# srsampson/SingleCarrier

Measured on AMD Instinct MI355X. Metric: demodulated Msamples/sec (whole node), 65536-channel 8 kHz batch; BER vs ref, higher is better.
Workload: dtype f32

## Files before the change

profiles/stamps.py:

```python
import ctypes as C
import json
import os
import sys

import numpy as np

ROOT = os.path.dirname(os.path.dirname(os.path.abspath(__file__)))
sys.path.insert(0, ROOT)
import singlecarrier_amd as sc

mode = sys.argv[1] if len(sys.argv) > 1 else "both"
if mode == "front":
    os.environ["QPSK_ABLATE"] = "front"
sc.LIB_PATH = os.path.join(ROOT, "singlecarrier_amd", "csrc", "build", "libqpsk_hip_stamps.so")
lib = sc.lib()
lib.qpsk_debug_stamps.argtypes = [C.c_void_p, C.c_int]
import torch

nch, nf = 65536, 32
x = torch.from_numpy(sc.synth(3, nch, nf)).cuda()
bits = torch.empty((nch, nf, 62), dtype=torch.uint8, device="cuda")
valid = torch.empty((nch, nf), dtype=torch.uint8, device="cuda")
rx = sc.Receiver(nch)
rx.demod_device(x, bits, valid)
torch.cuda.synchronize()
st = np.zeros(16, np.uint64)
lib.qpsk_debug_stamps(st.ctypes.data, 1)
rx.demod_device(x, bits, valid)
torch.cuda.synchronize()
lib.qpsk_debug_stamps(st.ctypes.data, 1)
names = {0: "mix", 1: "store_window+prefetch+sync", 6: "front_channel+mi+sync (total)",
         7: "frame barrier wait", 8: "FIR decimated (D)", 9: "FIR head (F)+sync",
         10: "T image+sync", 11: "correlate (MFMA)", 12: "argmax (DPP max)"}
bnames = {13: "back: frame (128 train steps + job/outputs)", 14: "back: frame barrier wait"}
ch_iters = nch * nf
waves = nch // 32
out = {"mode": mode, "cycles_per_channel": {}}
tot = sum(int(st[i]) for i in (0, 1, 6, 7))
for i, nm in names.items():
    v = int(st[i]) / ch_iters
    out["cycles_per_channel"][nm] = round(v, 1)
out["share_of_loop"] = {names[i]: round(int(st[i]) / tot, 3) for i in (0, 1, 6, 7)}
bw = nch // 64
btot = int(st[13]) + int(st[14])
out["back_cycles_per_frame"] = {bnames[i]: round(int(st[i]) / (bw * nf), 1) for i in (13, 14)}
out["back_share"] = {bnames[i]: round(int(st[i]) / max(btot, 1), 3) for i in (13, 14)}
fr = bw * nf
out["back_alone_tail"] = {
    "frames_back_last_share": round(int(st[5]) / fr, 3),
    "tail_cycles_per_frame_all": round(int(st[15]) / fr, 1),
    "tail_cycles_per_frame_when_last": round(int(st[15]) / max(int(st[5]), 1), 1),
    "frame_cycles": round(btot / fr, 1),
    "tail_share_of_frame": round(int(st[15]) / max(btot, 1), 3)}
print(json.dumps(out, indent=1))
```

singlecarrier_amd/__init__.py:

```python
from __future__ import annotations

import ctypes as C
import os
import subprocess

import numpy as np

HERE = os.path.dirname(os.path.abspath(__file__))
LIB_PATH = os.environ.get("QPSK_LIB") or os.path.join(HERE, "libqpsk_hip.so")

FRAME_SIZE = 1880
DATA_SYMBOLS = 31
PREAMBLE_LENGTH = 128
BITS_PER_FRAME = 496
NBITS = 62
CYCLES = 5

_lib = None


class _CF(C.Structure):
    _fields_ = [("re", C.c_float), ("im", C.c_float)]


class QpskError(RuntimeError):
    code = 0


QPSK_EINVAL, QPSK_ENOMEM, QPSK_ENODEV, QPSK_EBUSY, QPSK_ESTALL = -1, -2, -3, -4, -5


def build(verbose: bool = False) -> str:
    out = subprocess.run(["make", "-C", os.path.join(HERE, "csrc")], capture_output=True,
                         text=True)
    if out.returncode != 0:
        raise QpskError("build failed:\n" + out.stdout[-4000:] + out.stderr[-4000:])
    if verbose:
        print(out.stdout)
    return LIB_PATH


KERNEL_SOURCES = ("qpsk_rx.hip", "qpsk_rx_shared.h", "qpsk_herr.h", "qpsk_rx_dev.h", "qpsk_rx_front.h",
                  "qpsk_rx_back.h", "qpsk_rx_quad.h", "qpsk_hunt.h", "qpsk_rcp.h", "qpsk_consts.h",
                  "qpsk_fft_dev.h", "qpsk_split.h", "Makefile")


def kernel_source_hash(csrc: str = None) -> str:
    csrc = csrc or os.path.join(HERE, "csrc")
    inc = os.path.join(os.path.dirname(HERE), "include")
    out = subprocess.run(["make", "-s", "--no-print-directory", "-C", csrc, "khash", f"INCDIR={inc}"],
                         capture_output=True, text=True)
    if out.returncode != 0:
        raise QpskError("make khash failed:\n" + out.stderr[-2000:])
    return out.stdout.strip()


def kernel_hash() -> str:
    return lib().qpsk_kernel_hash().decode()


def lib():
    global _lib
    if _lib is None:
        if not os.path.exists(LIB_PATH):
            raise QpskError(f"{LIB_PATH} not built: run singlecarrier_amd.build() "
                            "or make -C singlecarrier_amd/csrc")
        try:
            import torch
        except Exception:
            pass
        L = C.CDLL(LIB_PATH)
        vp, i32, u64 = C.c_void_p, C.c_int, C.c_uint64
        L.qpsk_rx_create.restype = vp
        L.qpsk_rx_create.argtypes = [i32, i32, C.POINTER(C.c_int)]
        L.qpsk_rx_create_mode.restype = vp
        L.qpsk_rx_create_mode.argtypes = [i32, i32, i32, C.POINTER(C.c_int)]
        L.qpsk_rx_mode.argtypes = [vp]
        L.qpsk_rx_destroy.argtypes = [vp]
        L.qpsk_rx_reset.argtypes = [vp]
        L.qpsk_rx_channels.argtypes = [vp]
        L.qpsk_rx_frames.restype = u64
        L.qpsk_rx_frames.argtypes = [vp]
        L.qpsk_rx_batch.argtypes = [vp, vp, i32, vp, vp, vp, vp]
        L.qpsk_rx_batch_device.argtypes = [vp, vp, i32, vp, vp, vp, vp, vp]
        L.qpsk_strerror.restype = C.c_char_p
        L.qpsk_strerror.argtypes = [i32]
        L.qpsk_kernel_hash.restype = C.c_char_p
        L.qpsk_kernel_hash.argtypes = []
        L.qpsk_rx_frame.argtypes = [vp, vp]
        L.qpsk_tx_frame.argtypes = [vp, vp, i32, C.c_bool]
        L.qpsk_surface_error.restype = i32
        L.qpsk_rx_timing_enable.argtypes = [vp, i32]
        L.qpsk_rx_sync.argtypes = [vp]
        L.qpsk_rx_timing_collect.argtypes = [vp, C.POINTER(C.c_float), C.POINTER(C.c_int)]
        L.qpsk_rx_timing_split.argtypes = [vp, C.POINTER(C.c_float), C.POINTER(C.c_float),
# ... 432 lines not shown
```

singlecarrier_amd/csrc/qpsk_rx.hip:

```cpp

#if defined(QPSK_FRESH) || defined(QPSK_FRESH_SPLIT) || defined(QPSK_HUNT_MFMA) || \
    defined(QPSK_HUNT_FILTER) || defined(QPSK_HUNT_OVERLAP) || defined(QPSK_FIR_WAIT) || \
    defined(QPSK_FIR_ANCHOR) || defined(QPSK_FIR_SPLIT) || defined(QPSK_SPLIT_BANKS) || \
    defined(QPSK_QDMUL) || defined(QPSK_TRAIN_PRETAB) || defined(QPSK_DYNPRIO) || \
    defined(QPSK_DATA_RING) || defined(QPSK_LATE_YIELD) || defined(QPSK_FB) || defined(QPSK_FB1) || \
    defined(QPSK_ZERO_COPY)
#error "QPSK_FRESH, QPSK_FRESH_SPLIT, QPSK_HUNT_MFMA, QPSK_HUNT_FILTER, QPSK_HUNT_OVERLAP, QPSK_FIR_WAIT, QPSK_FIR_ANCHOR, QPSK_FIR_SPLIT, QPSK_SPLIT_BANKS, QPSK_QDMUL, QPSK_TRAIN_PRETAB, QPSK_DYNPRIO, QPSK_DATA_RING, QPSK_LATE_YIELD, QPSK_FB, QPSK_FB1 and QPSK_ZERO_COPY were removed with their alternative branches: DESIGN.md, Removed knobs, names the commit that still has each"
#endif

#include <hip/hip_runtime.h>

#include <stdint.h>

#include <algorithm>
#include <type_traits>

#include "qpsk_batch.h"
#include "qpsk_consts.h"
#include "qpsk_hunt.h"
#include "qpsk_rx_shared.h"
#include "qpsk_rx_dev.h"
#include "qpsk_rx_front.h"
#include "qpsk_rx_back.h"
#include "qpsk_rx_quad.h"

#pragma clang fp contract(off)

namespace {

#ifndef QPSK_RX_ATTR
#define QPSK_RX_ATTR
#endif
constexpr int kLateYield = 2;

template <int G, bool DUAL, int W, bool QUAD>
constexpr int kBackWavesOf = DUAL ? 2 * G * (QUAD ? W / 16 : 1) : G;

template <int G, int FP, bool DUAL, int W, bool QUAD>
constexpr int kWavesOf = kBackWavesOf<G, DUAL, W, QUAD> + G * FP;

template <int G, int FP, int MODE, bool DUAL, int W = QK_GROUP, bool QUAD = false, bool HP = false>
__global__ void __launch_bounds__((64 * kWavesOf<G, FP, DUAL, W, QUAD>),
                                  ((kWavesOf<G, FP, DUAL, W, QUAD> + 3) / 4)) QPSK_RX_ATTR rx_kernel(
    const int16_t* in, int16_t* hist, const float2* ptab, const unsigned long long* ks,
    float2* win0, float2* win1, int* mi0, int* mi1, int* rt0, int* rt1, uint8_t* bits,
    uint8_t* valid, int32_t* trace, float2* soft, float4* jobs, unsigned* njobs, int nch, int F,
    unsigned g0, int roles, const float* fft_tab, unsigned long long jcap, int* err) {
    static_assert(W == QK_GROUP || (DUAL && G == 1 && W % FP == 0 && W <= QK_GROUP), "group width");
    static_assert(!QUAD || (DUAL && G == 1 && W % 16 == 0), "quad backs: dual chain, one group");
    constexpr int kGroups = G, kFrontPer = FP;
    constexpr int kBackWaves = kBackWavesOf<G, DUAL, W, QUAD>;
    constexpr int kChainWaves = QUAD ? W / 16 : 1;
    constexpr bool kDyn = DUAL && QUAD;
    constexpr int kFrontCh = W / kFrontPer;
    constexpr int kFrontWaves = kGroups * kFrontPer;
    constexpr int kBlock = 64 * kWavesOf<G, FP, DUAL, W, QUAD>;
    const RxArgs a{in, hist, ptab, ks, win0, win1, mi0, mi1, rt0, rt1, bits, valid, trace, soft,
                   jobs, njobs, nch, F, g0, (size_t)jcap, roles, err,
                   HP ? reinterpret_cast<const float2*>(fft_tab) : nullptr};
    __shared__ __attribute__((aligned(16))) float2 P[QK_FRAME];
    constexpr int DM = MODE & 1;
    constexpr int kM = Cfg<DM>::kM, kDecBuf = Cfg<DM>::kDecBuf;
    __shared__ __attribute__((aligned(16))) float2 Ms[kFrontWaves][kM];
    __shared__ __attribute__((aligned(16))) float2 decs[kFrontWaves][kDecBuf][kDec];
    __shared__ int mi_s[kGroups][2][QK_GROUP], rt_s[kGroups][2][QK_GROUP];
    __shared__ __attribute__((aligned(16))) float BT[(MODE & 2) ? kFftHT : kHuntTab];
    constexpr bool kSplitK = MODE == 0 && !HP && !DUAL;
    __shared__ uint32_t p2w[kSplitK ? kSplitTabWords : 1];
    const uint8_t* p2tab = reinterpret_cast<const uint8_t*>(p2w);
    __shared__ int bseq[kGroups][2][kChainWaves], fcnt[kGroups][2][kChainWaves];
    __shared__ int dead_s;
    __shared__ int nwait_s;
#ifdef QPSK_STAMPS
    __shared__ unsigned long long tarr_s[16];
    __shared__ int tsimd_s[16];
#define TAIL_INIT() do { if (lane == 0 && wave < 16) tsimd_s[wave] = (int)((__builtin_amdgcn_s_getreg((31 << 11) | (0 << 6) | 4) >> 4) & 3); } while (0)
#define TAIL_ARRIVE() do { if (lane == 0 && wave < 16) tarr_s[wave] = stamp_now(); } while (0)
#define TAIL_BACK()                                                                           \
    do {                                                                                      \
        unsigned long long tf = 0;                                                            \
        for (int w2 = kBackWaves; w2 < kBackWaves + kFrontWaves && w2 < 16; w2++)             \
            if (tsimd_s[w2] == tsimd_s[wave] && tarr_s[w2] > tf) tf = tarr_s[w2];            \
        if (tf > 0 && tarr_s[wave] > tf) { st_acc[15] += tarr_s[wave] - tf; st_acc[5] += 1; } \
        st_t0 = stamp_now();                                                                  \
    } while (0)
#else
#define TAIL_INIT() do { } while (0)
#define TAIL_ARRIVE() do { } while (0)
#define TAIL_BACK() do { } while (0)
#endif
    if (blockDim.x != (unsigned)kBlock) {
        if (blockIdx.x == 0 && threadIdx.x == 0) atomicOr(err, kErrStall);
        return;
    }
    const int lane = threadIdx.x & 63;
    const int wave = __builtin_amdgcn_readfirstlane(threadIdx.x >> 6);
    const int grp0 = blockIdx.x * kGroups;
    TAIL_INIT();
    for (int i = threadIdx.x; i < QK_FRAME / 2; i += kBlock)
        reinterpret_cast<float4*>(P)[i] = reinterpret_cast<const float4*>(a.ptab)[i];
    if constexpr (kSplitK)
        for (int i = threadIdx.x; i < kSplitTabWords; i += kBlock)
            p2w[i] = reinterpret_cast<const uint32_t*>(&kSplitTab)[i];
    if constexpr ((MODE & 2) != 0) {
        for (int i = threadIdx.x; i < kFftHT; i += kBlock) BT[i] = fft_tab[i];
    } else {
        qhunt::bconst_h_lds(threadIdx.x, kBlock, BT);
    }
    if (wave < kGroups) {
        const int ch = (grp0 + wave) * W + lane;
        if (lane < W && ch < a.nch) {
            mi_s[wave][0][lane] = mi_of(a, a.g0)[ch];
            rt_s[wave][0][lane] = rt_of(a, a.g0)[ch];
        }
    }
    if (threadIdx.x < 2 * kGroups * kChainWaves) (&bseq[0][0][0])[threadIdx.x] = (&fcnt[0][0][0])[threadIdx.x] = 0;
    if (threadIdx.x == 0) dead_s = nwait_s = 0;
    __syncthreads();
    if constexpr (DUAL) {
        constexpr int kBlkCh = W / kChainWaves;
        constexpr int kFrontChB = kBlkCh / kFrontPer;
        static_assert(kBlkCh % kFrontPer == 0, "block split");
        if (wave < kBackWaves) {
            const int gi = (wave >> 1) / kChainWaves;
            const int b = (wave >> 1) % kChainWaves;
            const int sub = QUAD ? lane >> 2 : lane;
            const bool own = sub < kBlkCh;
            const int idx = kBlkCh * b + (own ? sub : 0);
            const int ch = (grp0 + gi) * W + idx;
            const bool live = own && ch < a.nch;
            if (kDyn || roles_prio(a.roles) == kPrioBack) __builtin_amdgcn_s_setprio(2);
            auto poll = [&] {
                if constexpr (kDyn) {
                    const int w = __builtin_amdgcn_readfirstlane(
                        __hip_atomic_load(&nwait_s, __ATOMIC_RELAXED, __HIP_MEMORY_SCOPE_WORKGROUP));
                    if (w > 0) __builtin_amdgcn_s_setprio(0);
                    else __builtin_amdgcn_s_setprio(2);
                }
            };
            if (roles_debug_stall(a.roles) && blockIdx.x == 0 && wave == 0)
                spin_wait(&fcnt[gi][0][0], 1 << 30, a.err, &dead_s, 1u << 12);
            STAMP_DECL
            for (int n = wave & 1; n < a.F; n += 2) {
                const int p = n & 1;
                if (n > 0) {
                    int* const fc = &fcnt[gi][p ^ 1][b];
                    const int need = kFrontPer * ((n - 1) / 2 + 1);
                    if constexpr (kDyn) {
                        const bool waits = __builtin_amdgcn_readfirstlane(__hip_atomic_load(
                                               fc, __ATOMIC_RELAXED, __HIP_MEMORY_SCOPE_WORKGROUP)) < need;
                        if (waits) {
                            __builtin_amdgcn_s_setprio(0);
                            if (lane == 0)
                                __hip_atomic_fetch_add(&nwait_s, 1, __ATOMIC_RELAXED, __HIP_MEMORY_SCOPE_WORKGROUP);
                        }
                        spin_wait(fc, need, a.err, &dead_s);
                        if (waits && lane == 0)
                            __hip_atomic_fetch_add(&nwait_s, -1, __ATOMIC_RELAXED, __HIP_MEMORY_SCOPE_WORKGROUP);
                    } else {
                        spin_wait(fc, need, a.err, &dead_s);
                    }
                }
                STAMP(14);
                const int mi = mi_s[gi][p][idx];
                auto get_rt = [&] {
                    STAMP(13);
                    if (n > 0) spin_wait(&bseq[gi][p ^ 1][b], (n - 1) / 2 + 1, a.err, &dead_s);
                    STAMP(15);
                    return rt_s[gi][p][idx];
                };
                const float2* wn = win_of(a, a.g0 + (unsigned)n) + (size_t)(live ? ch : 0) * kWinStride;
                int* rtn = own ? &rt_s[gi][p ^ 1][idx] : nullptr;
                if constexpr (QUAD)
                    back_frame_quad(a, live ? ch : 0, live, n, mi, get_rt, wn, rtn, poll);
                else
                    back_frame(a, live ? ch : 0, live, n, mi, get_rt, wn, rtn, poll);
                signal_add(&bseq[gi][p][b], 1, lane);
                STAMP(13);
            }
            STAMP_FLUSH();
        } else {
            const int f = wave - kBackWaves;
            const int gi = f / kFrontPer;
            const int fl = f % kFrontPer;
            const int split = (kGroups == 1 && kChainWaves == 1) ? roles_split(a.roles) : 0;
            auto share = [&](int x) { return ((x + kBackWaves) & 3) < kBackWaves; };
            int cbeg = 0;
            for (int x = 0; x < fl; x++) cbeg += kFrontChB + (share(x) ? -split : split);
            const int mych = kFrontChB + (share(fl) ? -split : split);
            auto bch0 = [&](int bb) { return (grp0 + gi) * W + kBlkCh * bb + cbeg; };
            auto blive = [&](int bb) { return max(0, min(mych, a.nch - bch0(bb))); };
            float2* M = Ms[f];
            int pf[kPf<DM>];
            constexpr bool kSplitD = false;
            if (kDyn) __builtin_amdgcn_s_setprio(1);
            else if (roles_prio(a.roles) == kPrioFront) __builtin_amdgcn_s_setprio(2);
            if (blive(0) > 0) prefetch<DM, false, kSplitD>(srcs(a, bch0(0), 0), lane, pf);
            STAMP_DECL
            int k = 0;
#define QPSK_DUAL_FRONT_FRAME(CG)                                                                              \
    do {                                                                                                       \
        const int p = n & 1;                                                                                   \
        const unsigned g = a.g0 + (unsigned)n;                                                                 \
        float2* wout = win_of(a, g + 1u);                                                                      \
        for (int bb = 0; bb < kChainWaves; bb++) {                                                             \
                                                  \
                                                   \
            if (n > 0) spin_wait(&bseq[gi][p ^ 1][bb], (n - 1) / 2 + 1, a.err, &dead_s);                       \
            STAMP(7);                                                                                          \
            const int c0 = bch0(bb), nl = (roles_front_idle(a.roles) && n >= 2) ? 0 : blive(bb);               \
            const int i0 = kBlkCh * bb + cbeg;                                                                 \
            int pmi = 0;                                                                                       \
            for (int c = 0; c < nl; c++, k++) {                                                                \
                const int ch = c0 + c;                                                                         \
                float2* dcur = decs[f][k % kDecBuf];                                                           \
                mix<DM, kSplitD>(lane, pf, g, P, M);                                                           \
                STAMP(0);                                                                                      \
                if (c > 0)                                                                                     \
                    store_window(lane, pmi, decs[f][(k - 1) % kDecBuf], wout + (size_t)(ch - 1) * kWinStride); \
                STAMP(4);                                                                                      \
                {                      \
                    int nb = bb, nc = c + 1, nn = n;                                                           \
                    if (nc >= nl) {                                                                            \
                        nc = 0;                                                                                \
                        nb = bb + 1;                                                                           \
                        while (nb < kChainWaves && blive(nb) == 0) nb++;                                       \
                        if (nb == kChainWaves) { nb = 0; nn = n + 1; }                                         \
                    }                                                                                          \
                    if (nn < a.F) prefetch<DM, CG, kSplitD>(srcs(a, bch0(nb) + nc, nn), lane, pf);             \
                }                                                                                              \
                wave_lds_sync();                                                                               \
                STAMP(1);                                                                                      \
                pmi = front_channel<MODE, HP, kSplitD>(lane, rt_s[gi][p][i0 + c], M, dcur, BT, p2tab,         \
                                              a.heads + ((size_t)ch * a.F + n) * kHeadOut FACC_ARG);           \
                if (lane == 0) mi_s[gi][p ^ 1][i0 + c] = pmi;                                                  \
                if (c + 1 == nl) store_window(lane, pmi, dcur, wout + (size_t)ch * kWinStride);                \
                wave_lds_sync();                                                                               \
                STAMP(6);                                                                                      \
            }                                                                                                  \
            signal_add(&fcnt[gi][p][bb], 1, lane);                                                             \
            STAMP(5);                                                                                          \
        }                                                                                                      \
    } while (0)
            if constexpr (QUAD) {
                auto frame_iter = [&](auto cg, int n) {
                    constexpr bool CG = decltype(cg)::value;
                    QPSK_DUAL_FRONT_FRAME(CG);
                };
                for (int n = 0; n < a.F && n < 2; n++) frame_iter(std::false_type{}, n);
                for (int n = 2; n < a.F; n++) frame_iter(std::true_type{}, n);
            } else {
                for (int n = 0; n < a.F; n++) QPSK_DUAL_FRONT_FRAME(false);
            }
#undef QPSK_DUAL_FRONT_FRAME
            STAMP_FLUSH();
            for (int bb = 0; bb < kChainWaves; bb++)
                carry_history<DM>(a.in, a.hist, a.F, bch0(bb), blive(bb), lane);
        }
        __syncthreads();
        if (wave < kBackWaves && (wave & 1) == 0) {
            const int gi = (wave >> 1) / kChainWaves;
            const int sub = QUAD ? lane >> 2 : lane;
            const int idx = kBlkCh * ((wave >> 1) % kChainWaves) + sub;
            const int ch = (grp0 + gi) * W + idx;
            if (sub < kBlkCh && ch < a.nch && (!QUAD || (lane & 3) == 0)) {
                const unsigned ge = a.g0 + (unsigned)a.F;
                mi_of(a, ge)[ch] = mi_s[gi][a.F & 1][idx];
                rt_of(a, ge)[ch] = rt_s[gi][a.F & 1][idx];
            }
        }
        return;
    }
    if (wave < kBackWaves) {
        const int gi = wave;
        const int ch = (grp0 + gi) * QK_GROUP + lane;
        const bool live = ch < a.nch;
        const bool any = (grp0 + gi) * QK_GROUP < a.nch;
        if (roles_prio(a.roles) == kPrioBack) __builtin_amdgcn_s_setprio(2);
        STAMP_DECL
        for (int n = 0; n < a.F; n++) {
            const int p = n & 1;
            if (any && roles_back(a.roles)) {
                const int rt = rt_s[gi][p][lane];
                back_frame(a, live ? ch : 0, live, n, mi_s[gi][p][lane], [=] { return rt; },
                           win_of(a, a.g0 + (unsigned)n) + (size_t)(live ? ch : 0) * kWinStride,
                           &rt_s[gi][p ^ 1][lane], [] {});
            }
            else
                rt_s[gi][p ^ 1][lane] = rt_s[gi][p][lane];
            STAMP(13);
            TAIL_ARRIVE();
            __syncthreads();
            STAMP(14);
            TAIL_BACK();
        }
        STAMP_FLUSH();
        if (live) {
            const unsigned ge = a.g0 + (unsigned)a.F;
            mi_of(a, ge)[ch] = mi_s[gi][a.F & 1][lane];
            rt_of(a, ge)[ch] = rt_s[gi][a.F & 1][lane];
        }
    } else {
        constexpr bool kSplit = MODE == 0 && !HP;
        const int f = wave - kBackWaves;
        const int gi = f / kFrontPer;
        const int cbeg = (f % kFrontPer) * kFrontCh;
        const int ch0 = (grp0 + gi) * QK_GROUP + cbeg;
        const int nlive = max(0, min(kFrontCh, a.nch - ch0));
        float2* M = Ms[f];
        const bool on = roles_front(a.roles) != 0 && nlive > 0;
        if (roles_prio(a.roles) == kPrioFront) __builtin_amdgcn_s_setprio(2);
        int pf[kPf<DM>];
        if (on) prefetch<DM, false, kSplit>(srcs(a, ch0, 0), lane, pf);
        STAMP_DECL
        for (int n = 0; n < a.F; n++) {
            const int p = n & 1;
            const unsigned g = a.g0 + (unsigned)n;
            float2* wout = win_of(a, g + 1u);
            int pmi = 0;
            for (int z = (f >= kFrontWaves / 2) ? roles_stagger(a.roles) : 0; z > 0; z--)
                __builtin_amdgcn_s_sleep(8);
            for (int c = 0; on && c < nlive; c++) {
                const int ch = ch0 + c;
                float2* dcur = decs[f][c % kDecBuf];
                if (c == nlive - kLateYield && roles_prio(a.roles) == kPrioFront)
                    __builtin_amdgcn_s_setprio(0);
                mix<DM, kSplit>(lane, pf, g, P, M);
                STAMP(0);
                if (c > 0) store_window(lane, pmi, decs[f][(c - 1) % kDecBuf], wout + (size_t)(ch - 1) * kWinStride);
                {
                    const bool same = c + 1 < nlive;
                    if (same || n + 1 < a.F)
                        prefetch<DM, false, kSplit>(srcs(a, same ? ch + 1 : ch0, same ? n : n + 1), lane, pf);
                }
                wave_lds_sync();
                STAMP(1);
                pmi = front_channel<MODE, HP, kSplit>(lane, rt_s[gi][p][cbeg + c], M, dcur, BT, p2tab,
                                              a.heads + ((size_t)ch * a.F + n) * kHeadOut FACC_ARG);
                if (lane == 0) mi_s[gi][p ^ 1][cbeg + c] = pmi;
                if (c + 1 == nlive) store_window(lane, pmi, dcur, wout + (size_t)ch * kWinStride);
                wave_lds_sync();
                STAMP(6);
            }
            TAIL_ARRIVE();
            __syncthreads();
            if (roles_prio(a.roles) == kPrioFront) __builtin_amdgcn_s_setprio(2);
            STAMP(7);
        }
        STAMP_FLUSH();
        carry_history<DM>(a.in, a.hist, a.F, ch0, nlive, lane);
    }
}

}

template <int KIND> struct ShapeOf;
template <int G_, int FP_, bool DUAL_, int W_, bool QUAD_> struct ShapeParams {
    static constexpr int G = G_, FP = FP_, W = W_;
    static constexpr bool DUAL = DUAL_, QUAD = QUAD_;
};
template <> struct ShapeOf<Shape::k4x2> : ShapeParams<4, 2, false, 64, false> {};
template <> struct ShapeOf<Shape::k2x4d> : ShapeParams<2, 4, true, 64, false> {};
template <> struct ShapeOf<Shape::k1x8d64> : ShapeParams<1, 8, true, 64, false> {};
template <> struct ShapeOf<Shape::k1x8q16> : ShapeParams<1, 8, true, 16, true> {};
template <> struct ShapeOf<Shape::k1x8q32> : ShapeParams<1, 8, true, 32, true> {};

template <int KIND, int MODE, bool HP>
static void launch_rx(const RxLaunch& a) {
    using S = ShapeOf<KIND>;
    constexpr size_t kPer = (size_t)S::G * S::W;
    constexpr int kBlock = 64 * kWavesOf<S::G, S::FP, S::DUAL, S::W, S::QUAD>;
    hipLaunchKernelGGL((rx_kernel<S::G, S::FP, MODE, S::DUAL, S::W, S::QUAD, HP>),
                       dim3((unsigned)((a.nch + kPer - 1) / kPer)), dim3(kBlock - a.short_block), 0,
                       a.s, a.in, a.hist, a.ptab, a.ks, a.win[0], a.win[1], a.mi[0],
                       a.mi[1], a.rt[0], a.rt[1], a.bits, a.valid, a.trace,
                       reinterpret_cast<float2*>(a.soft), a.jobs, a.njobs + a.parity, a.nch, a.F,
                       a.g0, a.roles, HP ? reinterpret_cast<const float*>(a.heads) : a.fft_tab,
                       (unsigned long long)a.jobs_cap, a.err);
}

template <int MODE, bool HP>
static void launch_shape(const RxLaunch& a) {
    switch (a.kind) {
        case Shape::k2x4d: return launch_rx<Shape::k2x4d, MODE, HP>(a);
        case Shape::k1x8d64: return launch_rx<Shape::k1x8d64, MODE, HP>(a);
        case Shape::k1x8q16: return launch_rx<Shape::k1x8q16, MODE, HP>(a);
        case Shape::k1x8q32: return launch_rx<Shape::k1x8q32, MODE, HP>(a);
        default: return launch_rx<Shape::k4x2, MODE, HP>(a);
    }
}

namespace {
__global__ void err_take_kernel(int* err) {
    if (threadIdx.x == 0) err[1] = atomicExch(&err[0], 0);
}
}

int qpsk_rx_take_err(int* d_err, hipStream_t s) {
    hipLaunchKernelGGL(err_take_kernel, dim3(1), dim3(64), 0, s, d_err);
    HCHECK(hipGetLastError());
    return QPSK_OK;
}

#ifndef QPSK_KERNEL_HASH
#define QPSK_KERNEL_HASH "unknown"
#endif
extern "C" const char* qpsk_kernel_hash(void) { return QPSK_KERNEL_HASH; }

#ifdef QPSK_STAMPS
extern "C" int qpsk_debug_stamps(unsigned long long* out16, int reset) {
    if (hipMemcpyFromSymbol(out16, HIP_SYMBOL(g_stamps), sizeof(unsigned long long) * 16) != hipSuccess)
        return -1;
    if (reset) {
        unsigned long long z[16] = {0};
        if (hipMemcpyToSymbol(HIP_SYMBOL(g_stamps), z, sizeof z) != hipSuccess) return -1;
    }
    return 0;
}
#endif

int qpsk_rx_launch_kernels(const RxLaunch& a) {
    if (a.hp) {
        const size_t ncf = (size_t)a.nch * (size_t)a.F;
        hipLaunchKernelGGL(head_kernel, dim3((unsigned)((ncf + 3) / 4)), dim3(256), 0, a.s, a.in,
                           a.hist, a.ptab, a.heads, a.nch, a.F,
                           a.g0);
        HCHECK(hipGetLastError());
        launch_shape<0, true>(a);
    } else {
        switch (a.mode) {
            case 0: launch_shape<0, false>(a); break;
            case 1: launch_shape<1, false>(a); break;
            case 2: launch_shape<2, false>(a); break;
            default: launch_shape<3, false>(a); break;
        }
    }
    HCHECK(hipGetLastError());
    if (a.ev_mid) HCHECK(hipEventRecord(a.ev_mid, a.s));
    const size_t need = (size_t)a.nch * (size_t)a.F;
    const unsigned dgrid = (unsigned)std::min<size_t>(kDataGrid, (need + kDataBlock - 1) / kDataBlock);
    hipLaunchKernelGGL(rx_data_kernel, dim3(dgrid), dim3(kDataBlock), 0, a.s, a.jobs,
                       (unsigned long long)a.jobs_cap, a.njobs, a.ks, a.bits,
                       reinterpret_cast<float2*>(a.soft), a.parity, a.roles & kForceExact, a.ctx_err,
                       a.err_to);
    HCHECK(hipGetLastError());
    if (a.ev_end) HCHECK(hipEventRecord(a.ev_end, a.s));
    return QPSK_OK;
}
```

singlecarrier_amd/csrc/qpsk_rx_dev.h:

```cpp
#pragma once

#include <hip/hip_runtime.h>

#include <stdint.h>

#include "qpsk_consts.h"
#include "qpsk_hunt.h"
#include "qpsk_rx_shared.h"

#pragma clang fp contract(off)

namespace {

constexpr int kDec = 296;
constexpr int kM1 = 1240;
template <int MODE> struct Cfg;
template <> struct Cfg<0> { static constexpr int kM = 1392, kDecBuf = 2; };
template <> struct Cfg<1> { static constexpr int kM = 1750, kDecBuf = 1; };

typedef float f2 __attribute__((ext_vector_type(2)));

constexpr unsigned long long kPreLo = qhunt::pre_mask(0), kPreHi = qhunt::pre_mask(1);

struct alignas(16) PreTab {
    float v[QK_NPRE];
};
constexpr PreTab make_pretab() {
    PreTab t{};
    for (int i = 0; i < QK_NPRE; i++) t.v[i] = ((i < 64 ? kPreLo >> i : kPreHi >> (i - 64)) & 1ull) ? 1.0f : -1.0f;
    return t;
}
__constant__ PreTab kPreTab = make_pretab();

struct RxArgs {
    const int16_t* in;
    int16_t* hist;
    const float2* ptab;
    const unsigned long long* ks;
    float2* win0;
    float2* win1;
    int* mi0;
    int* mi1;
    int* rt0;
    int* rt1;
    uint8_t* bits;
    uint8_t* valid;
    int32_t* trace;
    float2* soft;
    float4* jobs;
    unsigned* njobs;
    int nch, F;
    unsigned g0;
    size_t jcap;
    int roles;
    int* err;
    const float2* heads;
};

#ifdef QPSK_STAMPS
__device__ unsigned long long g_stamps[16];
#define STAMP_DECL unsigned long long st_acc[16] = {}; unsigned long long st_t0 = stamp_now();
#define STAMP(i) do { const unsigned long long t_ = stamp_now(); st_acc[i] += t_ - st_t0; st_t0 = t_; } while (0)
#define STAMP_FLUSH() do { if (lane == 0) for (int i_ = 0; i_ < 16; i_++) atomicAdd(&g_stamps[i_], st_acc[i_]); } while (0)
__device__ __forceinline__ unsigned long long stamp_now() {
    unsigned long long t;
    __builtin_amdgcn_sched_barrier(0);
    asm volatile("s_memtime %0\n\ts_waitcnt lgkmcnt(0)" : "=s"(t)::"memory");
    __builtin_amdgcn_sched_barrier(0);
    return t;
}
#else
#define STAMP_DECL
#define STAMP(i) do { } while (0)
#define STAMP_FLUSH() do { } while (0)
#endif

__device__ __forceinline__ float2* win_of(const RxArgs& a, unsigned g) { return (g & 1u) ? a.win1 : a.win0; }
__device__ __forceinline__ int* mi_of(const RxArgs& a, unsigned g) { return (g & 1u) ? a.mi1 : a.mi0; }
__device__ __forceinline__ int* rt_of(const RxArgs& a, unsigned g) { return (g & 1u) ? a.rt1 : a.rt0; }

__device__ __forceinline__ void wave_lds_sync() {
    __builtin_amdgcn_fence(__ATOMIC_RELEASE, "wavefront");
    __builtin_amdgcn_wave_barrier();
    __builtin_amdgcn_fence(__ATOMIC_ACQUIRE, "wavefront");
}

constexpr unsigned kSpinBound = 1u << 22;

__device__ __forceinline__ void spin_wait(int* p, int v, int* err, int* dead,
                                          unsigned bound = kSpinBound) {
    unsigned it = 0;
    for (; it < bound; it++) {
        const int c = __builtin_amdgcn_readfirstlane(
            __hip_atomic_load(p, __ATOMIC_RELAXED, __HIP_MEMORY_SCOPE_WORKGROUP));
        const int d = __builtin_amdgcn_readfirstlane(
            __hip_atomic_load(dead, __ATOMIC_RELAXED, __HIP_MEMORY_SCOPE_WORKGROUP));
        if (c >= v || d != 0) break;
        __builtin_amdgcn_s_sleep(1);
    }
    if (it == bound && __lane_id() == 0) {
        __hip_atomic_store(dead, 1, __ATOMIC_RELAXED, __HIP_MEMORY_SCOPE_WORKGROUP);
        atomicOr(err, kErrStall);
    }
    __builtin_amdgcn_fence(__ATOMIC_ACQUIRE, "workgroup");
}

__device__ __forceinline__ void signal_add(int* p, int v, int lane) {
    __builtin_amdgcn_fence(__ATOMIC_RELEASE, "workgroup");
    asm volatile("s_waitcnt vmcnt(0)" ::: "memory");
    if (lane == 0) __hip_atomic_fetch_add(p, v, __ATOMIC_RELAXED, __HIP_MEMORY_SCOPE_WORKGROUP);
}

__device__ __forceinline__ const int16_t* frame_ptr(const RxArgs& a, int ch, int k) {
    return k >= 0 ? a.in + ((size_t)ch * a.F + k) * QK_FRAME
                  : a.hist + ((size_t)ch * 2 + (k + 2)) * QK_FRAME;
}

}
```

singlecarrier_amd/csrc/qpsk_rx_front.h:

```cpp
#pragma once

#include <utility>

#include "qpsk_fft_dev.h"
#include "qpsk_rx_dev.h"
#include "qpsk_split.h"

#pragma clang fp contract(off)

namespace {

constexpr int kFirBatch = 15;

template <int MODE> constexpr int kItems = Cfg<MODE>::kM / 2;
template <int MODE> constexpr int kPf = (kItems<MODE> + 63) / 64;

struct Src {
    const int16_t* xm2;
    const int16_t* xm1;
    const int16_t* x0;
};

__device__ __forceinline__ Src srcs(const RxArgs& a, int ch, int n) {
    return {frame_ptr(a, ch, n - 2), frame_ptr(a, ch, n - 1), frame_ptr(a, ch, n)};
// ... 47 lines not shown
    prefetch_seq<MODE, CG>(s, (FR & 1) ? fresh_lane(lane) : lane, r, std::make_integer_sequence<int, kPf<MODE>>{});
}

template <int MODE, int i, bool NO>
__device__ __forceinline__ void mix_item(int lane, int r, const float2* P, float2* M) {
    int t;
    const int f = item<MODE, i>(lane, t);
    if (f < 0) return;
    const float4 p = *reinterpret_cast<const float4*>(P + t);
    const float v0 = (float)(int16_t)(r & 0xffff);
    const float v1 = (float)(int16_t)(r >> 16);
    float4 o;
    constexpr bool kAllPrev = MODE == 1 ? i >= 1 : (i >= 1 && i <= 9);
    if (kAllPrev) {
        o = NO ? make_float4((-p.x) * v0, (-p.y) * v0, (-p.z) * v1, (-p.w) * v1)
               : make_float4(p.x * v0, p.y * v0, p.z * v1, p.w * v1);
    } else {
        const float sg = ((f == 1) == NO) ? -1.0f : 1.0f;
        o = make_float4((sg * p.x) * v0, (sg * p.y) * v0, (sg * p.z) * v1, (sg * p.w) * v1);
    }
    *reinterpret_cast<float4*>(M + 2 * (lane + 64 * i)) = o;
}

template <int MODE, bool NO, int... I>
__device__ __forceinline__ void mix_seq(int lane, const int (&r)[kPf<MODE>], const float2* P,
                                        float2* M, std::integer_sequence<int, I...>) {
    (mix_item<MODE, I, NO>(lane, r[I], P, M), ...);
}

template <int MODE, int FR = 0>
__device__ __forceinline__ void mix(int lane, const int (&r)[kPf<MODE>], unsigned g,
                                    const float2* P, float2* M) {
    constexpr auto kSeq = std::make_integer_sequence<int, kPf<MODE>>{};
    if (FR & 2) lane = fresh_lane(lane);
    if (((g - 1u) & 1u) != 0) mix_seq<MODE, true>(lane, r, P, M, kSeq);
    else mix_seq<MODE, false>(lane, r, P, M, kSeq);
}

using qhunt::wave_max_u32;

typedef __attribute__((address_space(3))) const volatile f2 lds_vf2;
__device__ __forceinline__ f2 ld2nt(const float2* p) {
    return *(lds_vf2*)p;
}
__device__ __forceinline__ void anchor_f2(f2& y) { asm volatile("" : "+v"(y)); }
__device__ __forceinline__ void fir_batch_wait() {
    __builtin_amdgcn_sched_barrier(0);
    __builtin_amdgcn_s_waitcnt(0xC07F);
    __builtin_amdgcn_sched_barrier(0);
}

#ifdef QPSK_STAMPS
#define FSTAMP(i) do { const unsigned long long t_ = stamp_now(); facc[8 + (i)] += t_ - ft0; ft0 = t_; } while (0)
#define FACC_PARAM , unsigned long long (&facc)[16]
#define FACC_ARG , st_acc
#define FACC_FWD , facc
#else
#define FSTAMP(i) do { } while (0)
#define FACC_PARAM
#define FACC_ARG
#define FACC_FWD
#endif
__device__ __forceinline__ void fir_dec752(int lane, int rt, const float2* M, float2* dec) {
    if (lane < QK_NDECOBS / 5) {
        const float2* b = M + 25 * lane + rt;
        f2 y[5] = {{0.0f, 0.0f}, {0.0f, 0.0f}, {0.0f, 0.0f}, {0.0f, 0.0f}, {0.0f, 0.0f}};
#pragma unroll
        for (int s0 = 0; s0 < 69; s0 += kFirBatch) {
            f2 v[kFirBatch];
#pragma unroll
            for (int j = 0; j < kFirBatch; j++)
                if (s0 + j < 69) v[j] = ld2nt(b + s0 + j);
            fir_batch_wait();
#pragma unroll
            for (int j = 0; j < kFirBatch; j++) {
                const int s = s0 + j;
#pragma unroll
                for (int m = 0; m < 5; m++) {
                    const int k = s - 5 * m;
                    if (s < 69 && k >= 0 && k < QK_NTAPS) y[m] = y[m] + v[j] * QK_RRC[k];
                }
            }
        }
#pragma unroll
        for (int m = 0; m < 5; m++) {
            const f2 o = y[m] * QK_GAIN;
            dec[5 * lane + m] = make_float2(o.x, o.y);
        }
    }
}

constexpr int kHuntTab = qhunt::kBH + qhunt::kPL;
__device__ __forceinline__ int fft_hunt(int lane, float2* M, const float2* dec, const float* HT) {
    const qfft::cf* tw = reinterpret_cast<const qfft::cf*>(HT);
    const int* perm = reinterpret_cast<const int*>(HT + 768 * 2);
    qfft::cf* X = reinterpret_cast<qfft::cf*>(M);
    qfft::cf* Y = X + 256;
    const qfft::cf* d = reinterpret_cast<const qfft::cf*>(dec);
    for (int pos = lane; pos < 256; pos += 64) X[pos] = d[perm[pos]];
    qfft::lds_sync();
    qfft::stages(lane, 256, X, tw, false);
    for (int pos = lane; pos < 256; pos += 64) {
        const int k = perm[pos];
        Y[pos] = qfft::mul(X[k], tw[512 + k]);
    }
    qfft::lds_sync();
    qfft::stages(lane, 256, Y, tw + 256, true);
// ... 208 lines not shown
        fir_split(lane, rt, M, dec, p2tab);
        FSTAMP(0);
        wave_lds_sync();
        FSTAMP(1);
        const int mi = hunt<MODE>(lane, M, dec, BT FACC_FWD);
        if (mi >= kSplitMi) {
            fir_split_tail(lane, M, dec);
            wave_lds_sync();
        }
        return mi;
    } else {
        fir_dec(lane, rt, M, dec);
        FSTAMP(0);
        fir_head_at(lane, M + kM1, dec + QK_NDEC);
    }
    wave_lds_sync();
    FSTAMP(1);
    return hunt<MODE>(lane, M, dec, BT FACC_FWD);
}

__device__ __forceinline__ void store_window(int lane, int mi, const float2* dec, float2* out) {
    float4* o = reinterpret_cast<float4*>(out);
    {
        const float2 lo = dec[max(mi + 2 * lane - 1, 0)], hi = dec[mi + 2 * lane];
        o[lane] = make_float4(lo.x, lo.y, hi.x, hi.y);
    }
    if (lane < kWinStride / 2 - 64) {
        const int q = lane + 64;
        const float2 lo = dec[mi + 2 * q - 1], hi = dec[mi + 2 * q];
        o[q] = make_float4(lo.x, lo.y, hi.x, hi.y);
    }
}

template <int MODE>
__device__ __forceinline__ void carry_history(const int16_t* in, int16_t* hist, int F, int ch0, int nlive, int lane) {
    constexpr int kHead8 = MODE == 1 ? 213 : 149;
    for (int c = 0; c < nlive; c++) {
        const int ch = ch0 + c;
        int16_t* h0 = hist + (size_t)ch * 2 * QK_FRAME;
        int16_t* h1 = h0 + QK_FRAME;
        const int16_t* last = F >= 1 ? in + ((size_t)ch * F + (F - 1)) * QK_FRAME : h1;
        const int16_t* prev = F >= 2 ? in + ((size_t)ch * F + (F - 2)) * QK_FRAME : h1;
        if (lane < 6) {
            const int t = 1832 + 8 * lane;
            *reinterpret_cast<int4*>(h0 + t) = *reinterpret_cast<const int4*>(prev + t);
        }
        for (int u = lane; u < kHead8 + 6; u += 64) {
            const int t = u < kHead8 ? 8 * u : 1832 + 8 * (u - kHead8);
            *reinterpret_cast<int4*>(h1 + t) = *reinterpret_cast<const int4*>(last + t);
        }
    }
}

}
```

singlecarrier_amd/csrc/qpsk_rx_plan.h:

```cpp
#pragma once

#include <stddef.h>
#include <stdint.h>

#include "qpsk_consts.h"
#include "qpsk_rx_shared.h"

struct RxKnobs {
    int roles = roles_with_stagger(roles_with_prio(kRoleBack | kRoleFront, kPrioFront), kStagger);
    int shape = -1;
    int width = 0;
    int prio = -1;
    bool headpass = false;
    int stall_calls = -1;
    int short_block = 0;
};

inline Shape pick_shape(const RxKnobs& k, int nch, int ncu) {
    const int ngroup = (nch + QK_GROUP - 1) / QK_GROUP;
    Shape sh{k.shape, k.roles};
    if (sh.kind < 0)
        sh.kind = ngroup <= ncu ? Shape::k1x8d64 : ngroup <= 2 * ncu ? Shape::k2x4d : Shape::k4x2;
    if (sh.kind == Shape::k1x8d64) {
        const int W = k.width > 0 ? k.width
                    : (size_t)nch <= (size_t)16 * ncu ? 16
                    : (size_t)nch <= (size_t)32 * ncu ? 32 : 64;
        if (W == 16) sh.kind = Shape::k1x8q16;
        else if (W == 32) sh.kind = Shape::k1x8q32;
        else sh.roles = roles_with_split(roles_with_prio(sh.roles, kPrioBack), 2);
    }
    if (k.prio >= 0) sh.roles = roles_with_prio(sh.roles, k.prio);
    return sh;
}

struct Stage {
    size_t in, bits, valid, err, trace, soft, end;
};
inline Stage stage_of(size_t cf) {
    auto up = [](size_t x) { return (x + 255) & ~(size_t)255; };
    Stage g;
    g.in = 0;
    g.bits = up(sizeof(int16_t) * cf * QK_FRAME);
    g.valid = g.bits + cf * QK_NBITS;
    g.err = (g.valid + cf + 3) & ~(size_t)3;
    g.trace = up(g.err + sizeof(int));
    g.soft = up(g.trace + sizeof(int32_t) * cf * 4);
    g.end = up(g.soft + sizeof(float) * cf * QK_NDSYM * 2);
    return g;
}
constexpr size_t kPinnedStage = (size_t)8 << 20;
constexpr size_t kZeroCopyCF = 64;

struct StageView {
    char* base;
    Stage g;
    int16_t* in() const { return reinterpret_cast<int16_t*>(base + g.in); }
    uint8_t* bits() const { return reinterpret_cast<uint8_t*>(base + g.bits); }
    uint8_t* valid() const { return reinterpret_cast<uint8_t*>(base + g.valid); }
    int* err() const { return reinterpret_cast<int*>(base + g.err); }
    int32_t* trace() const { return reinterpret_cast<int32_t*>(base + g.trace); }
    float* soft() const { return reinterpret_cast<float*>(base + g.soft); }
};

constexpr char kStateMagic[8] = {'Q', 'P', 'S', 'K', 'S', 'T', 'A', '1'};
struct StateHdr {
    char magic[8];
    uint32_t version, hdr_bytes;
    int32_t mode, n;
    uint64_t frame;
    uint32_t hist_bytes, win_bytes;
    uint8_t pad[24];
};
static_assert(sizeof(StateHdr) == 64, "state header");
constexpr size_t kHistB = sizeof(int16_t) * 2 * QK_FRAME, kWinB = sizeof(float) * 2 * kWinStride;
constexpr size_t kChanB = kHistB + kWinB + 2 * sizeof(int);
constexpr int kWinObs = QK_NPRE + QK_NDSYM + 5;
static_assert(kWinObs == 164 && kWinObs <= kWinStride, "window slots");

inline size_t rx_state_size(int n) { return n < 1 ? 0 : sizeof(StateHdr) + (size_t)n * kChanB; }

inline size_t rx_nslot(int nch) {
    const int ngroup = (nch + QK_GROUP - 1) / QK_GROUP;
    return (size_t)((ngroup + kMaxGroups - 1) / kMaxGroups) * kMaxGroups * QK_GROUP;
}
```

Measured before the change: 673,900.

## Spread history carry across front frame loop instead of an epilogue pass

The per-channel history copy (last frame head/tail into the hist buffer) moves out of the post-loop epilogue. Each front wave now interleaves one channel's carry into its frame loop iterations, and in split mode issues the loads early alongside mix. This is meant to remove the serialized tail where front waves copy history after the loop while the workgroup idles. It adds register pressure and extra memory traffic inside the hot loop, and the carry is now restructured into separate load and store helpers. Epilogue and carry timing stamps are also added to the profiling script.

```diff
diff --git a/profiles/stamps.py b/profiles/stamps.py
--- a/profiles/stamps.py
+++ b/profiles/stamps.py
@@ -10,46 +10,82 @@
 import singlecarrier_amd as sc
 
 mode = sys.argv[1] if len(sys.argv) > 1 else "both"
+nch = int(sys.argv[2]) if len(sys.argv) > 2 else 65536
+nf = int(sys.argv[3]) if len(sys.argv) > 3 else 32
+calls = int(sys.argv[4]) if len(sys.argv) > 4 else 1
 if mode == "front":
     os.environ["QPSK_ABLATE"] = "front"
-sc.LIB_PATH = os.path.join(ROOT, "singlecarrier_amd", "csrc", "build", "libqpsk_hip_stamps.so")
+sc.LIB_PATH = os.environ.get("QPSK_STAMPS_LIB") or os.path.join(
+    ROOT, "singlecarrier_amd", "csrc", "build", "libqpsk_hip_stamps.so")
 lib = sc.lib()
 lib.qpsk_debug_stamps.argtypes = [C.c_void_p, C.c_int]
+lib.qpsk_debug_epilogue.argtypes = [C.c_void_p, C.c_int]
 import torch
 
-nch, nf = 65536, 32
-x = torch.from_numpy(sc.synth(3, nch, nf)).cuda()
+ncu = torch.cuda.get_device_properties(0).multi_processor_count
+x = sc.synth_device(3, nch, nf)
 bits = torch.empty((nch, nf, 62), dtype=torch.uint8, device="cuda")
 valid = torch.empty((nch, nf), dtype=torch.uint8, device="cuda")
 rx = sc.Receiver(nch)
 rx.demod_device(x, bits, valid)
-torch.cuda.synchronize()
+rx.sync()
 st = np.zeros(16, np.uint64)
+ep = np.zeros(4, np.uint64)
+lib.qpsk_debug_epilogue(ep.ctypes.data, 1)
 lib.qpsk_debug_stamps(st.ctypes.data, 1)
-rx.demod_device(x, bits, valid)
-torch.cuda.synchronize()
+rx.timing(True)
+rx.collect_timing()
+for _ in range(calls):
+    rx.demod_device(x, bits, valid)
+rx.sync()
+rx_ms, data_ms, _ = rx.collect_timing_split()
+lib.qpsk_debug_epilogue(ep.ctypes.data, 1)
 lib.qpsk_debug_stamps(st.ctypes.data, 1)
-names = {0: "mix", 1: "store_window+prefetch+sync", 6: "front_channel+mi+sync (total)",
-         7: "frame barrier wait", 8: "FIR decimated (D)", 9: "FIR head (F)+sync",
-         10: "T image+sync", 11: "correlate (MFMA)", 12: "argmax (DPP max)"}
-bnames = {13: "back: frame (128 train steps + job/outputs)", 14: "back: frame barrier wait"}
-ch_iters = nch * nf
-waves = nch // 32
-out = {"mode": mode, "cycles_per_channel": {}}
-tot = sum(int(st[i]) for i in (0, 1, 6, 7))
-for i, nm in names.items():
-    v = int(st[i]) / ch_iters
-    out["cycles_per_channel"][nm] = round(v, 1)
-out["share_of_loop"] = {names[i]: round(int(st[i]) / tot, 3) for i in (0, 1, 6, 7)}
-bw = nch // 64
-btot = int(st[13]) + int(st[14])
-out["back_cycles_per_frame"] = {bnames[i]: round(int(st[i]) / (bw * nf), 1) for i in (13, 14)}
-out["back_share"] = {bnames[i]: round(int(st[i]) / max(btot, 1), 3) for i in (13, 14)}
-fr = bw * nf
-out["back_alone_tail"] = {
-    "frames_back_last_share": round(int(st[5]) / fr, 3),
-    "tail_cycles_per_frame_all": round(int(st[15]) / fr, 1),
-    "tail_cycles_per_frame_when_last": round(int(st[15]) / max(int(st[5]), 1), 1),
-    "frame_cycles": round(btot / fr, 1),
-    "tail_share_of_frame": round(int(st[15]) / max(btot, 1), 3)}
+out = {"mode": mode, "channels": nch, "frames": nf, "calls": calls, "kernel_hash": sc.kernel_hash()}
+
+ngroup = (nch + 63) // 64
+if ngroup > 2 * ncu:
+    per_wg = 256
+elif ngroup > ncu:
+    per_wg = 128
+else:
+    per_wg = 16 if nch <= 16 * ncu else 32 if nch <= 32 * ncu else 64
+nwg = (nch + per_wg - 1) // per_wg
+fwaves = 8 * nwg
+rx_us = rx_ms / calls * 1e3
+e = [int(v) for v in ep]
+tail_share = e[1] / max(e[2], 1)
+out["epilogue"] = {
+    "workgroups": nwg, "front_waves": fwaves, "rx_kernel_us": round(rx_us, 2),
+    "carry_ticks_per_front_wave": round(e[0] / (fwaves * calls), 1),
+    "channels_carried_per_call": e[3] / calls,
+    "tail_ticks_per_workgroup (last wave out of the frame loop -> last exit)": round(e[1] / (nwg * calls), 1),
+    "workgroup_ticks (first start -> last exit)": round(e[2] / (nwg * calls), 1),
+    "carry_share_of_workgroup_time": round(e[0] / fwaves / max(e[2] / nwg, 1), 5),
+    "tail_share_of_workgroup_time": round(tail_share, 5),
+    "tail_us (share x rx_kernel_us)": round(tail_share * rx_us, 2)}
+
+if per_wg == 256:
+    names = {0: "mix", 1: "store_window+prefetch+sync", 6: "front_channel+mi+sync (total)",
+             7: "frame barrier wait", 8: "FIR decimated (D)", 9: "FIR head (F)+sync",
+             10: "T image+sync", 11: "correlate (MFMA)", 12: "argmax (DPP max)"}
+    bnames = {13: "back: frame (128 train steps + job/outputs)", 14: "back: frame barrier wait"}
+    ch_iters = nch * nf * calls
+    out["cycles_per_channel"] = {}
+    tot = sum(int(st[i]) for i in (0, 1, 6, 7))
+    for i, nm in names.items():
+        v = int(st[i]) / ch_iters
+        out["cycles_per_channel"][nm] = round(v, 1)
+    out["share_of_loop"] = {names[i]: round(int(st[i]) / tot, 3) for i in (0, 1, 6, 7)}
+    bw = nch // 64
+    btot = int(st[13]) + int(st[14])
+    out["back_cycles_per_frame"] = {bnames[i]: round(int(st[i]) / (bw * nf * calls), 1) for i in (13, 14)}
+    out["back_share"] = {bnames[i]: round(int(st[i]) / max(btot, 1), 3) for i in (13, 14)}
+    fr = bw * nf * calls
+    out["back_alone_tail"] = {
+        "frames_back_last_share": round(int(st[5]) / fr, 3),
+        "tail_cycles_per_frame_all": round(int(st[15]) / fr, 1),
+        "tail_cycles_per_frame_when_last": round(int(st[15]) / max(int(st[5]), 1), 1),
+        "frame_cycles": round(btot / fr, 1),
+        "tail_share_of_frame": round(int(st[15]) / max(btot, 1), 3)}
 print(json.dumps(out, indent=1))
diff --git a/singlecarrier_amd/__init__.py b/singlecarrier_amd/__init__.py
--- a/singlecarrier_amd/__init__.py
+++ b/singlecarrier_amd/__init__.py
@@ -40,7 +40,7 @@
     return LIB_PATH
 
 
-KERNEL_SOURCES = ("qpsk_rx.hip", "qpsk_rx_shared.h", "qpsk_herr.h", "qpsk_rx_dev.h", "qpsk_rx_front.h",
+KERNEL_SOURCES = ("qpsk_rx.hip", "qpsk_rx_shared.h", "qpsk_rx_plan.h", "qpsk_herr.h", "qpsk_rx_dev.h", "qpsk_rx_front.h",
                   "qpsk_rx_back.h", "qpsk_rx_quad.h", "qpsk_hunt.h", "qpsk_rcp.h", "qpsk_consts.h",
                   "qpsk_fft_dev.h", "qpsk_split.h", "Makefile")
 
diff --git a/singlecarrier_amd/csrc/qpsk_rx.hip b/singlecarrier_amd/csrc/qpsk_rx.hip
--- a/singlecarrier_amd/csrc/qpsk_rx.hip
+++ b/singlecarrier_amd/csrc/qpsk_rx.hip
@@ -19,6 +19,7 @@
 #include "qpsk_consts.h"
 #include "qpsk_hunt.h"
 #include "qpsk_rx_shared.h"
+#include "qpsk_rx_plan.h"
 #include "qpsk_rx_dev.h"
 #include "qpsk_rx_front.h"
 #include "qpsk_rx_back.h"
@@ -89,6 +90,7 @@
 #define TAIL_ARRIVE() do { } while (0)
 #define TAIL_BACK() do { } while (0)
 #endif
+    EPI_DECL
     if (blockDim.x != (unsigned)kBlock) {
         if (blockIdx.x == 0 && threadIdx.x == 0) atomicOr(err, kErrStall);
         return;
@@ -97,6 +99,7 @@
     const int wave = __builtin_amdgcn_readfirstlane(threadIdx.x >> 6);
     const int grp0 = blockIdx.x * kGroups;
     TAIL_INIT();
+    EPI_INIT();
     for (int i = threadIdx.x; i < QK_FRAME / 2; i += kBlock)
         reinterpret_cast<float4*>(P)[i] = reinterpret_cast<const float4*>(a.ptab)[i];
     if constexpr (kSplitK)
@@ -178,6 +181,7 @@
                 signal_add(&bseq[gi][p][b], 1, lane);
                 STAMP(13);
             }
+            EPI_LOOP_END();
             STAMP_FLUSH();
         } else {
             const int f = wave - kBackWaves;
@@ -253,9 +257,12 @@
                 for (int n = 0; n < a.F; n++) QPSK_DUAL_FRONT_FRAME(false);
             }
 #undef QPSK_DUAL_FRONT_FRAME
-            STAMP_FLUSH();
+            EPI_LOOP_END();
+            CARRY_T0();
             for (int bb = 0; bb < kChainWaves; bb++)
                 carry_history<DM>(a.in, a.hist, a.F, bch0(bb), blive(bb), lane);
+            CARRY_T1(blive(0) + (kChainWaves > 1 ? blive(1) : 0));
+            STAMP_FLUSH();
         }
         __syncthreads();
         if (wave < kBackWaves && (wave & 1) == 0) {
@@ -269,6 +276,7 @@
                 rt_of(a, ge)[ch] = rt_s[gi][a.F & 1][idx];
             }
         }
+        EPI_EXIT(kBlock / 64);
         return;
     }
     if (wave < kBackWaves) {
@@ -294,6 +302,7 @@
             STAMP(14);
             TAIL_BACK();
         }
+        EPI_LOOP_END();
         STAMP_FLUSH();
         if (live) {
             const unsigned ge = a.g0 + (unsigned)a.F;
@@ -302,6 +311,8 @@
         }
     } else {
         constexpr bool kSplit = MODE == 0 && !HP;
+        constexpr bool kCarryEarly = kSplit;
+        constexpr bool kCarryLoop = MODE != 2;
         const int f = wave - kBackWaves;
         const int gi = f / kFrontPer;
         const int cbeg = (f % kFrontPer) * kFrontCh;
@@ -318,6 +329,7 @@
             const unsigned g = a.g0 + (unsigned)n;
             float2* wout = win_of(a, g + 1u);
             int pmi = 0;
+            int cnext = kCarryLoop ? carry_first(n, a.F) : -1;
             for (int z = (f >= kFrontWaves / 2) ? roles_stagger(a.roles) : 0; z > 0; z--)
                 __builtin_amdgcn_s_sleep(8);
             for (int c = 0; on && c < nlive; c++) {
@@ -325,9 +337,19 @@
                 float2* dcur = decs[f][c % kDecBuf];
                 if (c == nlive - kLateYield && roles_prio(a.roles) == kPrioFront)
                     __builtin_amdgcn_s_setprio(0);
+                const bool cy = kCarryLoop && c == cnext;
+                CarryRegs cr;
+                if (kCarryEarly && cy) carry_load<DM>(a.in, a.hist, a.F, ch, lane, cr);
                 mix<DM, kSplit>(lane, pf, g, P, M);
                 STAMP(0);
                 if (c > 0) store_window(lane, pmi, decs[f][(c - 1) % kDecBuf], wout + (size_t)(ch - 1) * kWinStride);
+                if (cy) {
+                    CARRY_T0();
+                    if (!kCarryEarly) carry_load<DM>(a.in, a.hist, a.F, ch, lane, cr);
+                    carry_store<DM>(a.hist, ch, lane, cr);
+                    cnext += carry_step(a.F);
+                    CARRY_T1(1);
+                }
                 {
                     const bool same = c + 1 < nlive;
                     if (same || n + 1 < a.F)
@@ -347,9 +369,15 @@
             if (roles_prio(a.roles) == kPrioFront) __builtin_amdgcn_s_setprio(2);
             STAMP(7);
         }
+        EPI_LOOP_END();
+        if constexpr (!kCarryLoop) {
+            CARRY_T0();
+            carry_history<DM>(a.in, a.hist, a.F, ch0, nlive, lane);
+            CARRY_T1(nlive);
+        }
         STAMP_FLUSH();
-        carry_history<DM>(a.in, a.hist, a.F, ch0, nlive, lane);
-    }
+    }
+    EPI_EXIT(kBlock / 64);
 }
 
 }
@@ -414,6 +442,15 @@
     if (reset) {
         unsigned long long z[16] = {0};
         if (hipMemcpyToSymbol(HIP_SYMBOL(g_stamps), z, sizeof z) != hipSuccess) return -1;
+    }
+    return 0;
+}
+extern "C" int qpsk_debug_epilogue(unsigned long long* out4, int reset) {
+    const size_t off = sizeof(unsigned long long) * 16, len = sizeof(unsigned long long) * (kStamps - 16);
+    if (hipMemcpyFromSymbol(out4, HIP_SYMBOL(g_stamps), len, off) != hipSuccess) return -1;
+    if (reset) {
+        unsigned long long z[kStamps - 16] = {0};
+        if (hipMemcpyToSymbol(HIP_SYMBOL(g_stamps), z, len, off) != hipSuccess) return -1;
     }
     return 0;
 }
diff --git a/singlecarrier_amd/csrc/qpsk_rx_dev.h b/singlecarrier_amd/csrc/qpsk_rx_dev.h
--- a/singlecarrier_amd/csrc/qpsk_rx_dev.h
+++ b/singlecarrier_amd/csrc/qpsk_rx_dev.h
@@ -58,10 +58,11 @@
 };
 
 #ifdef QPSK_STAMPS
-__device__ unsigned long long g_stamps[16];
-#define STAMP_DECL unsigned long long st_acc[16] = {}; unsigned long long st_t0 = stamp_now();
+constexpr int kStamps = 20;
+__device__ unsigned long long g_stamps[kStamps];
+#define STAMP_DECL unsigned long long st_acc[kStamps] = {}; unsigned long long st_t0 = stamp_now();
 #define STAMP(i) do { const unsigned long long t_ = stamp_now(); st_acc[i] += t_ - st_t0; st_t0 = t_; } while (0)
-#define STAMP_FLUSH() do { if (lane == 0) for (int i_ = 0; i_ < 16; i_++) atomicAdd(&g_stamps[i_], st_acc[i_]); } while (0)
+#define STAMP_FLUSH() do { if (lane == 0) for (int i_ = 0; i_ < kStamps; i_++) atomicAdd(&g_stamps[i_], st_acc[i_]); } while (0)
 __device__ __forceinline__ unsigned long long stamp_now() {
     unsigned long long t;
     __builtin_amdgcn_sched_barrier(0);
@@ -69,10 +70,37 @@
     __builtin_amdgcn_sched_barrier(0);
     return t;
 }
+struct EpiClock {
+    unsigned long long start, loop_end, exit;
+    int exited;
+};
+#define EPI_DECL __shared__ EpiClock epi_s;
+#define EPI_INIT() do { if (threadIdx.x == 0) { epi_s.start = stamp_now(); epi_s.loop_end = epi_s.exit = 0; epi_s.exited = 0; } } while (0)
+#define EPI_LOOP_END() do { if (lane == 0) atomicMax(&epi_s.loop_end, stamp_now()); } while (0)
+#define EPI_EXIT(nwaves)                                                                  \
+    do {                                                                                  \
+        if (lane == 0) {                                                                  \
+            atomicMax(&epi_s.exit, stamp_now());                                          \
+            __threadfence_block();                                                        \
+            if (atomicAdd(&epi_s.exited, 1) == (nwaves) - 1) {                            \
+                const unsigned long long te_ = atomicMax(&epi_s.exit, 0ull);              \
+                atomicAdd(&g_stamps[17], te_ - atomicMax(&epi_s.loop_end, 0ull));         \
+                atomicAdd(&g_stamps[18], te_ - epi_s.start);                              \
+            }                                                                             \
+        }                                                                                 \
+    } while (0)
+#define CARRY_T0() const unsigned long long ct0_ = stamp_now()
+#define CARRY_T1(n) do { st_acc[16] += stamp_now() - ct0_; st_acc[19] += (n); } while (0)
 #else
+#define CARRY_T0() do { } while (0)
+#define CARRY_T1(n) do { } while (0)
 #define STAMP_DECL
 #define STAMP(i) do { } while (0)
 #define STAMP_FLUSH() do { } while (0)
+#define EPI_DECL
+#define EPI_INIT() do { } while (0)
+#define EPI_LOOP_END() do { } while (0)
+#define EPI_EXIT(nwaves) do { } while (0)
 #endif
 
 __device__ __forceinline__ float2* win_of(const RxArgs& a, unsigned g) { return (g & 1u) ? a.win1 : a.win0; }
diff --git a/singlecarrier_amd/csrc/qpsk_rx_front.h b/singlecarrier_amd/csrc/qpsk_rx_front.h
--- a/singlecarrier_amd/csrc/qpsk_rx_front.h
+++ b/singlecarrier_amd/csrc/qpsk_rx_front.h
@@ -123,7 +123,7 @@
 
 #ifdef QPSK_STAMPS
 #define FSTAMP(i) do { const unsigned long long t_ = stamp_now(); facc[8 + (i)] += t_ - ft0; ft0 = t_; } while (0)
-#define FACC_PARAM , unsigned long long (&facc)[16]
+#define FACC_PARAM , unsigned long long (&facc)[kStamps]
 #define FACC_ARG , st_acc
 #define FACC_FWD , facc
 #else
@@ -438,4 +438,53 @@
     }
 }
 
-}
+template <int MODE> struct CarryCfg {
+    static constexpr int kHead8 = MODE == 1 ? 213 : 149;
+    static constexpr int kTail = kHead8 + 6, kAll = kHead8 + 12, kPer = (kAll + 63) / 64;
+    static_assert((kPer == 3 || kPer == 4) && 64 * (kPer - 1) <= kHead8, "tails in the last unit of a lane");
+};
+typedef int i4 __attribute__((ext_vector_type(4)));
+struct CarryRegs {
+    i4 v0, v1, v2, vl;
+};
+template <int MODE>
+__device__ __forceinline__ int carry_last_unit(int lane, bool& pv) {
+    using K = CarryCfg<MODE>;
+    const int ul = min(lane + 64 * (K::kPer - 1), K::kAll - 1);
+    pv = ul >= K::kTail;
+    return ul < K::kHead8 ? 8 * ul : 1832 + 8 * (ul - (pv ? K::kTail : K::kHead8));
+}
+
+template <int MODE>
+__device__ __forceinline__ void carry_load(const int16_t* in, const int16_t* hist, int F, int ch, int lane,
+                                           CarryRegs& r) {
+    asm volatile("" : "+s"(ch), "+s"(F));
+    lane = fresh_lane(lane);
+    const int16_t* last = in + ((size_t)ch * F + (F - 1)) * QK_FRAME;
+    const int16_t* prev = F >= 2 ? last - QK_FRAME : hist + ((size_t)ch * 2 + 1) * QK_FRAME;
+    bool pv;
+    const int tl = carry_last_unit<MODE>(lane, pv);
+    __builtin_amdgcn_sched_barrier(0);
+    r.v0 = *reinterpret_cast<const i4*>(last + 8 * lane);
+    r.v1 = *reinterpret_cast<const i4*>(last + 8 * (lane + 64));
+    if (CarryCfg<MODE>::kPer > 3) r.v2 = *reinterpret_cast<const i4*>(last + 8 * (lane + 128));
+    r.vl = *reinterpret_cast<const i4*>((pv ? prev : last) + tl);
+    __builtin_amdgcn_sched_barrier(0);
+}
+
+template <int MODE>
+__device__ __forceinline__ void carry_store(int16_t* hist, int ch, int lane, const CarryRegs& r) {
+    asm volatile("" : "+s"(ch));
+    lane = fresh_lane(lane);
+    int16_t* h0 = hist + (size_t)ch * 2 * QK_FRAME;
+    bool pv;
+    const int tl = carry_last_unit<MODE>(lane, pv);
+    __builtin_amdgcn_sched_barrier(0);
+    *reinterpret_cast<i4*>(h0 + QK_FRAME + 8 * lane) = r.v0;
+    *reinterpret_cast<i4*>(h0 + QK_FRAME + 8 * (lane + 64)) = r.v1;
+    if (CarryCfg<MODE>::kPer > 3) *reinterpret_cast<i4*>(h0 + QK_FRAME + 8 * (lane + 128)) = r.v2;
+    *reinterpret_cast<i4*>(h0 + (pv ? 0 : QK_FRAME) + tl) = r.vl;
+    __builtin_amdgcn_sched_barrier(0);
+}
+
+}
diff --git a/singlecarrier_amd/csrc/qpsk_rx_plan.h b/singlecarrier_amd/csrc/qpsk_rx_plan.h
--- a/singlecarrier_amd/csrc/qpsk_rx_plan.h
+++ b/singlecarrier_amd/csrc/qpsk_rx_plan.h
@@ -32,6 +32,10 @@
     if (k.prio >= 0) sh.roles = roles_with_prio(sh.roles, k.prio);
     return sh;
 }
+
+constexpr int carry_iter(int c, int F) { return F >= 2 ? 1 + c % (F - 1) : 0; }
+constexpr int carry_step(int F) { return F >= 2 ? F - 1 : 1; }
+constexpr int carry_first(int n, int F) { return F >= 2 ? n - 1 : 0; }
 
 struct Stage {
     size_t in, bits, valid, err, trace, soft, end;
```

After: 677,800 (median of 6 runs). About the same (+0.6%).
